# ByeongKyuPark/Depth-Aware-Shader-Effects-for-NeRF

Hardware: AMD Instinct MI355X
Metric: rays/sec at 800x800, 64 coarse + 128 fine samples (higher is better)
Workload: dtype fp32 (f16x3 split)

## Files before the change

### depth-aware-shader-effects-for-nerf_amd/csrc/mlp16s.hip

```cpp
#include <atomic>
#include "common.h"
#include "pe_sin.h"
#include "stream16.h"

namespace nerf {

#ifdef NERF_MLP16S_STAMPS
__device__ unsigned long long nerf16s_stamps[65536][16];
constexpr int kSStampFloats = kW16Waves * 32;
constexpr int kSStampIter = 8;
#define STAMP16S_ASM(i, insn)                                                               \
  do {                                                                                      \
    __builtin_amdgcn_sched_barrier(0);                                                      \
    unsigned long long t_;                                                                  \
    asm volatile(insn " %0\n\ts_waitcnt lgkmcnt(0)" : "=s"(t_)::"memory");                 \
    __builtin_amdgcn_sched_barrier(0);                                                      \
    if (lane == 0 && stamp_on) reinterpret_cast<unsigned long long*>(lds + kSLdsFloats)[wave * 16 + (i)] = t_; \
  } while (0)
#define STAMP16S(i) STAMP16S_ASM(i, "s_memtime")
#define STAMP16S_REAL(i) STAMP16S_ASM(i, "s_memrealtime")
#else
constexpr int kSStampFloats = 0;
#define STAMP16S(i) do {} while (0)
#define STAMP16S_REAL(i) do {} while (0)
#endif

__device__ __forceinline__ f32x4 mfma16s(h16x8 a, h16x8 b, f32x4 c) {
  return __builtin_amdgcn_mfma_f32_16x16x32_f16(a, b, c, 0, 0, 0);
}

constexpr int kSLdsPe = 4 * kChunkFloats;
constexpr int kSLdsBias = kSLdsPe + kW16Waves * kPeSteps * 64;
constexpr int kSLdsSigmaW = kSLdsBias + 8 * kHidden;
constexpr int kSLdsVecFloats = 8 * kHidden + kHidden + 4;
constexpr int kSLdsConsts = kSLdsBias + kSLdsVecFloats;
constexpr int kSLdsRgb = kSLdsConsts + kS16Consts;
constexpr int kSLdsRgbFloats = 3 * kDirHidden + 4;
constexpr int kSLdsFeat = kSLdsRgb + kSLdsRgbFloats;
constexpr int kSLdsFloats = kSLdsFeat + kW16Waves * kRayFeat;
static_assert(kSLdsRgb % 4 == 0 && kSLdsFeat % 4 == 0, "LDS vector layout");
static_assert((kS16Chunks & (kS16Chunks - 1)) == 0 && kS16Chunks % 4 == 0, "the stream wraps onto the same ring slots");

typedef h16x8 STile[2][2];
typedef f32x4 SAcc[8][2][2];

template <int TI>
__device__ __forceinline__ void sread_tile(const float* slot, const uint32_t (&off)[2], STile& a) {
#pragma unroll
  for (int r = 0; r < 2; ++r)
#pragma unroll
    for (int part = 0; part < 2; ++part)
      a[r][part] = __builtin_bit_cast(h16x8, *reinterpret_cast<const f32x4*>(slot + off[r] + TI * 512 + part * 256));
}

template <int G, int TI, bool FIRST, typename Hook>
__device__ __forceinline__ void smfma_tile(const STile& a, const Operand& b0, const Operand& b1, SAcc& acc,
                                           Hook&& hook) {
  static_for<4>([&](auto jc) __attribute__((always_inline)) {
    constexpr int j = decltype(jc)::value, r = j >> 1, st = j & 1;
    const Operand& b = st ? b1 : b0;
    f32x4 c;
    if constexpr (FIRST) c = mfma16s(a[r][1], b.hi, f32x4{});
    else c = mfma16s(a[r][1], b.hi, acc[4 * G + TI][r][st]);
    c = mfma16s(a[r][0], b.lo, c);
    acc[4 * G + TI][r][st] = mfma16s(a[r][0], b.hi, c);
    hook(jc);
  });
}

constexpr int kSValuGap0 = 5;
template <int G, int TI, bool FIRST, int NRD, int VPG, typename Reads, typename Side, typename Hook>
__device__ __forceinline__ void ssegment(const STile& a, const Operand& b0, const Operand& b1, SAcc& acc, Reads&& reads,
                                         Side&& side, Hook&& hook) {
  side(std::integral_constant<int, 0>{});
  __builtin_amdgcn_sched_barrier(0);
  reads();
  smfma_tile<G, TI, FIRST>(a, b0, b1, acc, hook);
  side(std::integral_constant<int, 1>{});
#pragma unroll
  for (int i = 0; i < 12; ++i) {
    __builtin_amdgcn_sched_group_barrier(0x008, 1, 0);
    if (i >= 1 && i <= 4 * NRD) __builtin_amdgcn_sched_group_barrier(0x100, 1, 0);
    if (VPG > 0 && i >= kSValuGap0) __builtin_amdgcn_sched_group_barrier(0x002, VPG, 0);
  }
  __builtin_amdgcn_sched_barrier(0);
}

enum SSide { kSNone, kSPrev, kSCur, kSL0, kSSkipPrev, kSSkipCur, kSPrevPe, kSCurPe };
__device__ __forceinline__ constexpr int spe_at(int i, int seg) {
  return (i == 7 || i == 8) && (seg == 0 || seg == 2) ? 2 * (i - 7) + seg / 2 : -1;
}
__device__ __forceinline__ constexpr int sq_prev(int i, int seg) {
  constexpr int base[7] = {0, 3, 6, 8, 10, 12, 14};
  if (i >= 7) return -1;
  const int n = i < 2 ? 3 : 2;
  if (n == 3) return seg >= 1 ? base[i] + seg - 1 : -1;
  return seg == 1 ? base[i] : (seg == 3 ? base[i] + 1 : -1);
}
__device__ __forceinline__ constexpr int sq_cur(int i, int seg) {
  constexpr int base[8] = {0, 0, 2, 4, 6, 8, 11, 14};
  constexpr int cnt[8] = {0, 2, 2, 2, 2, 3, 3, 2};
  if (i >= 8 || cnt[i] == 0) return -1;
  if (cnt[i] == 3) return seg >= 1 ? base[i] + seg - 1 : -1;
  return seg == 1 ? base[i] : (seg == 3 ? base[i] + 1 : -1);
}
template <bool CUR>
__device__ __forceinline__ constexpr int spe_next(int i, int seg) {
  if (i >= 8 || (CUR ? sq_cur(i, seg) : sq_prev(i, seg)) >= 0) return -1;
  int n = 0;
  for (int k = 0; k < 4 * i + seg; ++k) n += (CUR ? sq_cur(k / 4, k % 4) : sq_prev(k / 4, k % 4)) < 0;
  return n + (CUR ? 0 : 16);
}
static_assert(spe_next<true>(7, 2) == 15 && spe_next<false>(7, 3) == 31, "32 free segments");
template <int KIND>
__device__ __forceinline__ constexpr int side_count(int i, int seg) {
  if constexpr (KIND == kSPrevPe || KIND == kSCurPe) return 1;
  if constexpr (KIND == kSPrev) return sq_prev(i, seg) >= 0;
  if constexpr (KIND == kSSkipPrev) return (sq_prev(i, seg) >= 0) + (spe_at(i, seg) >= 0);
  if constexpr (KIND == kSCur) return sq_cur(i, seg) >= 0;
  if constexpr (KIND == kSSkipCur) return (sq_cur(i, seg) >= 0) + (spe_at(i, seg) >= 0);
  if constexpr (KIND == kSL0) return 2;
  return 0;
}
template <int KIND>
__device__ __forceinline__ constexpr int svpg(int i, int seg) {
  const int n = side_count<KIND>(i, seg);
  return n == 0 ? 0 : (n * 40 + 11 - kSValuGap0) / (12 - kSValuGap0);
}

struct SNoPub {
  template <typename I>
  __device__ __forceinline__ void operator()(I) const {}
};
template <int G, int SLOT, bool FIRST, int TAIL, int KIND, int I, bool WRAP, typename Side, typename Pub>
__device__ __forceinline__ void schunk(const float* __restrict__ stream, int c, float* lds, uint32_t lds_dma,
                                       uint32_t voff, const uint32_t (&off)[2], STile (&a)[4], const Operand& b0,
                                       const Operand& b1, SAcc& acc, Side&& side, Pub&& pub) {
  const float* cur = lds + SLOT * kChunkFloats;
  const float* nxt = lds + ((SLOT + 1) & 3) * kChunkFloats;
  auto none = [](auto) {};
  auto sd = [&side](auto seg_c) __attribute__((always_inline)) {
    return [&side, seg_c](auto ph) __attribute__((always_inline)) { side(std::integral_constant<int, I>{}, seg_c, ph); };
  };
  using S0 = std::integral_constant<int, 0>;
  using S1 = std::integral_constant<int, 1>;
  using S2 = std::integral_constant<int, 2>;
  using S3 = std::integral_constant<int, 3>;
  ssegment<G, 0, FIRST, 1, svpg<KIND>(I, 0)>(a[0], b0, b1, acc, [&]() __attribute__((always_inline)) {
    sread_tile<3>(cur, off, a[3]);
  }, sd(S0{}), none);
  if constexpr (TAIL >= 1) {
    wait_vmcnt<TAIL >= 2 ? 4 : 0>();
    __builtin_amdgcn_s_barrier();
  }
  pub(std::integral_constant<int, I>{});
  auto dma = [&](auto pc) __attribute__((always_inline)) {
    if constexpr (TAIL >= 3)
      chunk_dma_piece<(SLOT + 3) & 3, decltype(pc)::value>(stream, WRAP ? (c + 3) & (kS16Chunks - 1) : c + 3, lds_dma,
                                                           voff);
  };
  ssegment<G, 1, FIRST, (TAIL >= 1), svpg<KIND>(I, 1)>(a[1], b0, b1, acc, [&]() __attribute__((always_inline)) {
    if constexpr (TAIL >= 1) sread_tile<0>(nxt, off, a[0]);
  }, sd(S1{}), [&](auto jc) __attribute__((always_inline)) {
    if constexpr (decltype(jc)::value == 0) dma(S0{});
    if constexpr (decltype(jc)::value == 2) dma(S1{});
  });
  ssegment<G, 2, FIRST, (TAIL >= 1), svpg<KIND>(I, 2)>(a[2], b0, b1, acc, [&]() __attribute__((always_inline)) {
    if constexpr (TAIL >= 1) sread_tile<1>(nxt, off, a[1]);
  }, sd(S2{}), [&](auto jc) __attribute__((always_inline)) {
    if constexpr (decltype(jc)::value == 0) dma(S2{});
  });
  ssegment<G, 3, FIRST, (TAIL >= 1), svpg<KIND>(I, 3)>(a[3], b0, b1, acc, [&]() __attribute__((always_inline)) {
    if constexpr (TAIL >= 1) sread_tile<2>(nxt, off, a[2]);
  }, sd(S3{}), [&](auto jc) __attribute__((always_inline)) {
    if constexpr (decltype(jc)::value == 0) dma(S3{});
  });
}

template <int G, int NSTEP, int SLOT0, int TAIL_END, int KIND, bool WRAP = false, typename Opnd, typename Side,
          typename Pub = SNoPub>
__device__ __forceinline__ void sgroup(const float* __restrict__ stream, int c0, float* lds, uint32_t lds_dma,
                                       uint32_t voff, const uint32_t (&off)[2], STile (&a)[4], SAcc& acc,
                                       Opnd&& operand, Side&& side, Pub&& pub = Pub{}) {
  static_for<NSTEP>([&](auto ic) __attribute__((always_inline)) {
    constexpr int i = decltype(ic)::value;
    constexpr int left = NSTEP - 1 - i + TAIL_END;
    schunk<G, (SLOT0 + i) & 3, i == 0, (left < 3 ? left : 3), KIND, i, WRAP>(
        stream, c0 + i, lds, lds_dma, voff, off, a, operand(ic, std::integral_constant<int, 0>{}),
        operand(ic, std::integral_constant<int, 1>{}), acc, side, pub);
  });
}

__device__ __forceinline__ float smax4(float m) {
  m = fmaxf(m, __shfl_xor(m, 16));
  return fmaxf(m, __shfl_xor(m, 32));
}
__device__ __forceinline__ float ssum4(float v) {
  v = v + __shfl_xor(v, 16);
  return v + __shfl_xor(v, 32);
}

struct SQuarter {
  f32x4 b, w;
};

template <int PH, int T0, int QG, bool SIGMA>
__device__ __forceinline__ void squarter(const SAcc& acc, const float (&inv)[2], const float* bias, const float* ws,
                                         int nlane, const float (&sc)[2], Operand (&in)[16], float (&m)[2],
                                         float (&part)[2], SQuarter& qv) {
  constexpr int T = T0 + QG / 4, r = (QG % 4) >> 1, st = QG & 1;
  const int n0 = 32 * T + 8 * r + nlane;
  if constexpr (PH == 0) {
    qv.b = *reinterpret_cast<const f32x4*>(bias + n0);
    if constexpr (SIGMA) qv.w = *reinterpret_cast<const f32x4*>(ws + n0);
  } else {
    float xs[4];
#pragma unroll
    for (int e = 0; e < 4; ++e) {
      const float y = fmaxf(fmaf(acc[T][r][st][e], inv[st], qv.b[e]), 0.0f);
      m[st] = fmaxf(m[st], y);
      if constexpr (SIGMA) part[st] = fmaf(qv.w[e], y, part[st]);
      xs[e] = y * sc[st];
    }
    Operand& op = in[2 * T + st];
    typedef _Float16 h16x2 __attribute__((ext_vector_type(2)));
#pragma unroll
    for (int p = 0; p < 2; ++p) {
      const h16x2 hi2 = {(_Float16)xs[2 * p], (_Float16)xs[2 * p + 1]};
      const h16x2 lo2 = __builtin_bit_cast(h16x2, split_lo_pair(__builtin_bit_cast(uint32_t, hi2), xs[2 * p], xs[2 * p + 1]));
      const int j = 4 * r + 2 * p;
      op.hi[j] = hi2[0];
      op.hi[j + 1] = hi2[1];
      op.lo[j] = lo2[0];
      op.lo[j + 1] = lo2[1];
    }
  }
}

template <int PH, int t, int st>
__device__ __forceinline__ void spe_operand(const float* pe_mine, const float (&sc)[2], Operand& op, float (&v)[8],
                                            int lane) {
  if constexpr (PH == 0) {
#pragma unroll
    for (int j = 0; j < 8; ++j) v[j] = pe_mine[((st * 2 + t) * 8 + j) * 64 + lane];
  } else {
#pragma unroll
    for (int j = 0; j < 8; ++j) split_into(v[j] * sc[st], op, j);
  }
}

#define MLP16S_GATHER 0
#include "mlp16s_body.h"
#undef MLP16S_GATHER
#define MLP16S_GATHER 1
#include "mlp16s_body.h"
#undef MLP16S_GATHER

static int device_cus() {
  static std::atomic<int> cached[64];
  int dev = 0;
  if (hipGetDevice(&dev) != hipSuccess || dev < 0 || dev >= 64) return 0;
  int n = cached[dev].load(std::memory_order_relaxed);
  if (n == 0) {
    if (hipDeviceGetAttribute(&n, hipDeviceAttributeMultiprocessorCount, dev) != hipSuccess || n <= 0) return 0;
    cached[dev].store(n, std::memory_order_relaxed);
  }
  return n;
}

int launch_mlp16s(const float* packed, const float* o, const float* d, const float* z, int64_t R, int N,
                  const float* feat, float* rgb, float* sigma, const int* out_slot, int out_T, hipStream_t s) {
  const int64_t M = R * (int64_t)N;
  if (M == 0) return NERF_OK;
  constexpr int per_block = 32 * kW16Waves;
  const int64_t blocks = (M + per_block - 1) / per_block;
  const int cus = device_cus();
  if (cus <= 0) return set_error(NERF_ERR_HIP, "mlp16s_kernel: cannot read the device's CU count");
  hipLaunchKernelGGL(mlp16s_kernel, dim3((unsigned)(blocks < cus ? blocks : cus)), dim3(64 * kW16Waves), 0, s, packed, o, d, z, M, N, feat,
                     rgb, sigma, out_slot, out_T);
  return check_launch("mlp16s_kernel");
}

int launch_mlp16s_live(const float* packed, const float* o, const float* d, const float* z, int64_t R, int N,
                       const float* feat, float* rgb, float* sigma, const int* live, const int* live_count,
                       hipStream_t s) {
  const int64_t M = R * (int64_t)N;
  if (M == 0) return NERF_OK;
  constexpr int per_block = 32 * kW16Waves;
  const int64_t blocks = (M + per_block - 1) / per_block;
  const int cus = device_cus();
  if (cus <= 0) return set_error(NERF_ERR_HIP, "mlp16s_live_kernel: cannot read the device's CU count");
  hipLaunchKernelGGL(mlp16s_live_kernel, dim3((unsigned)(blocks < cus ? blocks : cus)), dim3(64 * kW16Waves), 0, s,
                     packed, o, d, z, N, feat, rgb, sigma, live, live_count);
  return check_launch("mlp16s_live_kernel");
}

}
```

### depth-aware-shader-effects-for-nerf_amd/csrc/mlp16s_body.h

```cpp
__global__ void __launch_bounds__(64 * kW16Waves, 1)
#if MLP16S_GATHER
mlp16s_live_kernel(const float* __restrict__ packed, const float* __restrict__ orig, const float* __restrict__ dirs,
                   const float* __restrict__ zv, int N, const float* __restrict__ feat, float* __restrict__ rgb,
                   float* __restrict__ sigma, const int* __restrict__ live, const int* __restrict__ live_count) {
#else
mlp16s_kernel(const float* __restrict__ packed, const float* __restrict__ orig, const float* __restrict__ dirs,
              const float* __restrict__ zv, int64_t M, int N, const float* __restrict__ feat,
              float* __restrict__ rgb, float* __restrict__ sigma, const int* __restrict__ out_slot, int out_T) {
#endif
  __shared__ __attribute__((aligned(16))) float lds[kSLdsFloats + kSStampFloats];
  const int wave = __builtin_amdgcn_readfirstlane(threadIdx.x >> 6), lane0 = threadIdx.x & 63;
#if MLP16S_GATHER
  const int64_t M = *live_count;
  if ((int64_t)blockIdx.x * (32 * kW16Waves) >= M) return;
  const int* const out_slot = nullptr;
  constexpr int out_T = 0;
#endif
  const int mlast = (int)(M - 1);
  const int nblk = (int)((M + 32 * kW16Waves - 1) / (32 * kW16Waves));
  int blk = blockIdx.x;
  auto sample_of = [&](int b, int st) {
    return imin64(((int64_t)b * kW16Waves + wave) * 32 + 16 * st + (lane0 & 15), (int64_t)mlast);
  };
  float in_z[2], in_o[2][3], in_d[2][3];
#if MLP16S_GATHER
  int sm_cur[2], sm_n[2];
  auto load_live = [&](int b, int (&sm)[2]) __attribute__((always_inline)) {
#pragma unroll
    for (int st = 0; st < 2; ++st) sm[st] = live[sample_of(b, st)];
  };
  auto load_inputs = [&](const int (&sml)[2]) __attribute__((always_inline)) {
#pragma unroll
    for (int st = 0; st < 2; ++st) {
      const int sm = sml[st];
#else
  auto load_inputs = [&](int b) __attribute__((always_inline)) {
#pragma unroll
    for (int st = 0; st < 2; ++st) {
      const int sm = (int)sample_of(b, st);
#endif
      const int64_t row = zv ? sm / N : sm;
#pragma unroll
      for (int c = 0; c < 3; ++c) in_o[st][c] = orig[3 * row + c];
      in_z[st] = 0.0f;
#pragma unroll
      for (int c = 0; c < 3; ++c) in_d[st][c] = 0.0f;
      if (zv) {
        in_z[st] = zv[sm];
#pragma unroll
        for (int c = 0; c < 3; ++c) in_d[st][c] = dirs[3 * row + c];
      }
    }
  };
  float x[2][3];
  auto positions = [&](float (&x)[2][3]) __attribute__((always_inline)) {
#pragma unroll
    for (int st = 0; st < 2; ++st)
#pragma unroll
      for (int c = 0; c < 3; ++c) {
        const float p = in_o[st][c] + in_d[st][c] * in_z[st];
        x[st][c] = zv ? p : in_o[st][c];
      }
  };
#if MLP16S_GATHER
  load_live(blk, sm_cur);
  load_inputs(sm_cur);
#else
  load_inputs(blk);
#endif
  positions(x);
  for (int i = threadIdx.x; i < kSLdsVecFloats / 4; i += 64 * kW16Waves)
    reinterpret_cast<f32x4*>(lds + kSLdsBias)[i] = reinterpret_cast<const f32x4*>(packed + kOffBias)[i];
  if (threadIdx.x < kS16Consts) lds[kSLdsConsts + threadIdx.x] = packed[kOffScale16 + threadIdx.x];
  if (threadIdx.x < kSLdsRgbFloats / 4)
    reinterpret_cast<f32x4*>(lds + kSLdsRgb)[threadIdx.x] = reinterpret_cast<const f32x4*>(packed + kOffRgbW)[threadIdx.x];
  __builtin_amdgcn_s_waitcnt(0);
  __builtin_amdgcn_sched_barrier(0);
  const float* stream = packed + kOff16;
  uint32_t lds_dma = (uint32_t)(uintptr_t)(lptr_t)lds + 1024u * wave;
  auto fragment_offsets = [](int l, uint32_t (&off)[2]) __attribute__((always_inline)) {
    const int li = l & 15, hh = (l >> 4) & 1, ss = l >> 5;
#pragma unroll
    for (int r = 0; r < 2; ++r) off[r] = (uint32_t)(ss * 2048 + 4 * ((li & 7) + 8 * r + 16 * (li >> 3) + 32 * hh));
  };
  float* pe_mine = lds + kSLdsPe + wave * kPeSteps * 64;
  const float* bias = lds + kSLdsBias;
  const float* ws = lds + kSLdsSigmaW;
  const float* cst = lds + kSLdsConsts;
#if MLP16S_GATHER
  constexpr bool one_ray = false;
#else
  const bool one_ray = (N & 31) == 0;
#endif
  float* feat_mine = lds + kSLdsFeat + wave * kRayFeat;
  STile a[4];
  {
    const uint32_t voff = 16u * lane0 + 1024u * wave;
    chunk_dma<0>(stream, 0, lds_dma, voff);
    chunk_dma<1>(stream, 1, lds_dma, voff);
    chunk_dma<2>(stream, 2, lds_dma, voff);
    uint32_t off[2];
    fragment_offsets(lane0, off);
    wait_vmcnt<8>();
    __builtin_amdgcn_s_barrier();
    sread_tile<0>(lds, off, a[0]);
    sread_tile<1>(lds, off, a[1]);
    sread_tile<2>(lds, off, a[2]);
  }

  Operand pe_op[4];
  bool full = true;
#ifdef NERF_MLP16S_STAMPS
  int it = 0;
#endif
#pragma unroll 1
  for (;;) {
  asm volatile("" : "+s"(stream));
  asm volatile("" : "+s"(lds_dma));
  int lane = lane0;
  asm volatile("" : "+v"(lane));
  const int g = lane >> 4, li = lane & 15, hh = g & 1, ss = g >> 1;
  const uint32_t voff = 16u * lane + 1024u * wave;
  uint32_t off[2];
  fragment_offsets(lane, off);
  const int nlane = 4 * hh + 16 * ss;
#ifdef NERF_MLP16S_STAMPS
  const bool stamp_on = it == kSStampIter || (it < kSStampIter && blk + (int)gridDim.x >= nblk);
  ++it;
#endif
  STAMP16S(0);
  STAMP16S_REAL(12);
  const int64_t s0 = ((int64_t)blk * kW16Waves + wave) * 32;

  auto pe_arg = [&](const float (&xa)[2][3], int st, int p) __attribute__((always_inline)) {
    const int fi = p / 3, fc = p - 3 * fi;
    const float xc = fc == 0 ? xa[st][0] : (fc == 1 ? xa[st][1] : xa[st][2]);
    return xc * __int_as_float((127 + (fi < kPosLevels ? fi : 0)) << 23);
  };
  auto pe_tail = [&](const float (&xa)[2][3], int st, int p, float v) __attribute__((always_inline)) {
    return p < 3 * kPosLevels ? v : (p == 30 ? (hh ? xa[st][1] : xa[st][0]) : (hh ? 0.0f : xa[st][2]));
  };
  auto pe_beyond = [&](const float (&xa)[2][3]) __attribute__((always_inline)) {
    float ax = 0.0f;
#pragma unroll
    for (int st = 0; st < 2; ++st)
      ax = fmaxf(ax, fmaxf(fabsf(xa[st][0]), fmaxf(fabsf(xa[st][1]), fabsf(xa[st][2]))));
    return __any(ax * (float)(1 << (kPosLevels - 1)) > kPeSinMax) != 0;
  };
  auto pe_bound = [&](const float (&xa)[2][3], int st) __attribute__((always_inline)) {
    return fmaxf(1.0f, fmaxf(fabsf(xa[st][0]), fmaxf(fabsf(xa[st][1]), fabsf(xa[st][2]))));
  };
  float m_pe[2];
  float s_cur[2], inv_cur[2], s_nxt[2], inv_prev[2], m[2] = {0.0f, 0.0f}, part[2] = {0.0f, 0.0f};
#pragma unroll
  for (int st = 0; st < 2; ++st) {
    m_pe[st] = pe_bound(x, st);
    s_cur[st] = pow2_scale(m_pe[st]);
  }
  if (full) {
    float pe[2][2][8];
    if (pe_beyond(x)) {
#pragma unroll
      for (int st = 0; st < 2; ++st)
#pragma unroll
        for (int t = 0; t < 2; ++t)
#pragma unroll
          for (int j = 0; j < 8; ++j) {
            const int p = 8 * (2 * t + ss) + j;
            float sn, cs;
            sincosf(pe_arg(x, st, p), &sn, &cs);
            pe[st][t][j] = pe_tail(x, st, p, hh ? cs : sn);
          }
    } else {
#pragma unroll
      for (int st = 0; st < 2; ++st)
#pragma unroll
        for (int t = 0; t < 2; ++t)
#pragma unroll
          for (int j = 0; j < 8; ++j) {
            const int p = 8 * (2 * t + ss) + j;
            pe[st][t][j] = pe_tail(x, st, p, pe_sin_reduced(pe_arg(x, st, p), hh));
          }
    }
#pragma unroll
    for (int st = 0; st < 2; ++st)
#pragma unroll
      for (int t = 0; t < 2; ++t)
#pragma unroll
        for (int j = 0; j < 8; ++j) {
          pe_mine[((st * 2 + t) * 8 + j) * 64 + lane] = pe[st][t][j];
          split_into(pe[st][t][j] * s_cur[st], pe_op[2 * t + st], j);
        }
  }
  const int nxt_blk = blk + (int)gridDim.x;
  float xn[2][3], s_n[2];
  bool beyond_n = false;
  Operand pe_nx[4];
  int lane_n = lane;
  auto pub_next = [&](auto ic) __attribute__((always_inline)) {
#if MLP16S_GATHER
    if constexpr (decltype(ic)::value == 0) load_live(nxt_blk, sm_n);
    if constexpr (decltype(ic)::value == 1) load_inputs(sm_n);
    if constexpr (decltype(ic)::value == 3) {
#else
    if constexpr (decltype(ic)::value == 0) load_inputs(nxt_blk);
    if constexpr (decltype(ic)::value == 2) {
#endif
      asm volatile("" : "+v"(lane_n));
      positions(xn);
#pragma unroll
      for (int st = 0; st < 2; ++st) s_n[st] = pow2_scale(pe_bound(xn, st));
      beyond_n = pe_beyond(xn);
    }
  };
  auto side_pe_next = [&](auto nc, auto ph) __attribute__((always_inline)) {
    constexpr int n = decltype(nc)::value;
    if constexpr (n >= 0 && decltype(ph)::value == 1) {
      constexpr int st = n >> 4, t = (n >> 3) & 1, j = n & 7;
      constexpr int p0 = 16 * t + j, p1 = p0 + 8;
      constexpr int f0 = p0 / 3, c0 = p0 % 3, f1 = p1 / 3 < kPosLevels ? p1 / 3 : 0, c1 = p1 % 3;
      const bool upper = lane_n >= 32;
      const int hn = (lane_n >> 4) & 1;
      const float a0 = xn[st][c0] * (float)(1 << f0), a1 = xn[st][c1] * (float)(1 << f1);
      const float r = pe_sin_reduced(upper ? a1 : a0, hn);
      float v = r;
      if constexpr (p1 == 30) v = upper ? (hn ? xn[st][1] : xn[st][0]) : r;
      if constexpr (p1 == 31) v = upper ? (hn ? 0.0f : xn[st][2]) : r;
      pe_mine[((st * 2 + t) * 8 + j) * 64 + lane_n] = v;
      split_into(v * s_n[st], pe_nx[2 * t + st], j);
      asm volatile("" : "+v"(pe_nx[2 * t + st].hi), "+v"(pe_nx[2 * t + st].lo));
    }
  };
  SAcc acc;
  Operand in[16];
#pragma unroll
  for (int st = 0; st < 2; ++st) {
    inv_cur[st] = cst[kS16InvW + 0] / s_cur[st];
    s_nxt[st] = pow2_scale(cst[kS16R + 0] * m_pe[st] + cst[kS16B + 0]);
  }
  SQuarter qv[2];
  float pe_v[8];
  auto pe_operand_of = [&](auto i, auto st) -> const Operand& {
    return pe_op[2 * decltype(i)::value + decltype(st)::value];
  };

  STAMP16S(1);
  sgroup<0, 2, 0, 3, kSNone>(stream, 0, lds, lds_dma, voff, off, a, acc, pe_operand_of,
                             [](auto, auto, auto) {});
  sgroup<1, 2, 2, 3, kSL0>(stream, 2, lds, lds_dma, voff, off, a, acc, pe_operand_of,
                           [&](auto i, auto seg, auto ph) __attribute__((always_inline)) {
                             constexpr int q0 = 8 * decltype(i)::value + 2 * decltype(seg)::value;
                             squarter<decltype(ph)::value, 0, q0, false>(acc, inv_cur, bias, ws, nlane, s_nxt, in, m,
                                                                         part, qv[0]);
                             squarter<decltype(ph)::value, 0, q0 + 1, false>(acc, inv_cur, bias, ws, nlane, s_nxt, in,
                                                                             m, part, qv[1]);
                           });

  STAMP16S(2);
#pragma unroll
  for (int st = 0; st < 2; ++st) {
    inv_prev[st] = inv_cur[st];
    s_cur[st] = s_nxt[st];
  }
  const float* bias_prev = bias;
  auto act_operand = [&](auto i, auto st) -> const Operand& { return in[2 * decltype(i)::value + decltype(st)::value]; };
  auto op4 = [&](auto i, auto st) -> const Operand& {
    constexpr int k = decltype(i)::value, t = decltype(st)::value;
    if constexpr (k < 8) return in[2 * k + t];
    else return pe_op[2 * (k - 8) + t];
  };
  auto side_prev = [&](auto i, auto seg, auto ph, auto sigma_tag) __attribute__((always_inline)) {
    constexpr int q = sq_prev(decltype(i)::value, decltype(seg)::value);
    if constexpr (q >= 0)
      squarter<decltype(ph)::value, 4, q, decltype(sigma_tag)::value>(acc, inv_prev, bias_prev, ws, nlane, s_cur, in, m,
                                                                       part, qv[0]);
  };
  auto side_cur = [&](auto i, auto seg, auto ph, const float* bias_l, auto sigma_tag) __attribute__((always_inline)) {
    constexpr int q = sq_cur(decltype(i)::value, decltype(seg)::value);
    if constexpr (q >= 0)
      squarter<decltype(ph)::value, 0, q, decltype(sigma_tag)::value>(acc, inv_cur, bias_l, ws, nlane, s_nxt, in, m,
                                                                      part, qv[1]);
  };
  float s_pe[2] = {0.0f, 0.0f};
  auto side_pe = [&](auto i, auto seg, auto ph) __attribute__((always_inline)) {
    constexpr int k = spe_at(decltype(i)::value, decltype(seg)::value);
    if constexpr (k >= 0) spe_operand<decltype(ph)::value, k / 2, k % 2>(pe_mine, s_pe, pe_op[k], pe_v, lane);
  };
  using NoSigma = std::false_type;
  using Sigma = std::true_type;
  auto layer = [&](int L, auto skip_tag, auto sg_tag, auto&& pub_a) __attribute__((always_inline)) {
    constexpr bool SKIP = decltype(skip_tag)::value;
    constexpr bool SG = decltype(sg_tag)::value;
#pragma unroll
    for (int st = 0; st < 2; ++st) {
      inv_cur[st] = cst[kS16InvW + L] / s_cur[st];
      if constexpr (SKIP) s_pe[st] = s_cur[st];
    }
    const float* bias_l = bias + L * kHidden;
    const int c0 = s16_chunk0(1) + (L - 1) * 16 + (L > kSkipLayer ? 4 : 0);
    if constexpr (SKIP) {
      sgroup<0, 10, 0, 3, kSSkipPrev>(stream, c0, lds, lds_dma, voff, off, a, acc, op4,
                                      [&](auto i, auto seg, auto ph) __attribute__((always_inline)) {
                                        side_prev(i, seg, ph, NoSigma{});
                                        side_pe(i, seg, ph);
                                      });
    } else {
      sgroup<0, 8, 0, 3, kSPrev>(stream, c0, lds, lds_dma, voff, off, a, acc, act_operand,
                                 [&](auto i, auto seg, auto ph) __attribute__((always_inline)) {
                                   side_prev(i, seg, ph, NoSigma{});
                                 }, pub_a);
    }
#pragma unroll
    for (int st = 0; st < 2; ++st) {
      const float ms = smax4(m[st]);
      float bound = cst[kS16R + L] * (SKIP ? fmaxf(ms, m_pe[st]) : ms) + cst[kS16B + L];
      if (L + 1 == kSkipLayer) bound = fmaxf(bound, m_pe[st]);
      s_nxt[st] = pow2_scale(bound);
      m[st] = 0.0f;
    }
    if constexpr (SKIP) {
      sgroup<1, 10, 2, 3, kSSkipCur>(stream, c0 + 10, lds, lds_dma, voff, off, a, acc, op4,
                                     [&](auto i, auto seg, auto ph) __attribute__((always_inline)) {
                                       side_cur(i, seg, ph, bias_l, NoSigma{});
                                       side_pe(i, seg, ph);
                                     });
    } else {
      sgroup<1, 8, 0, 3, SG ? kSCurPe : kSCur>(
          stream, c0 + 8, lds, lds_dma, voff, off, a, acc, act_operand,
          [&](auto i, auto seg, auto ph) __attribute__((always_inline)) {
            side_cur(i, seg, ph, bias_l, sg_tag);
            if constexpr (SG)
              side_pe_next(std::integral_constant<int, spe_next<true>(decltype(i)::value, decltype(seg)::value)>{}, ph);
          });
    }
#pragma unroll
    for (int st = 0; st < 2; ++st) {
      inv_prev[st] = inv_cur[st];
      s_cur[st] = s_nxt[st];
    }
    bias_prev = bias_l;
    STAMP16S(2 + L);
  };
#pragma unroll 1
  for (int L = 1; L < kSkipLayer; ++L) layer(L, NoSigma{}, NoSigma{}, SNoPub{});
  layer(kSkipLayer, Sigma{}, NoSigma{}, SNoPub{});
#pragma unroll 1
  for (int L = kSkipLayer + 1; L < 7; ++L) layer(L, NoSigma{}, NoSigma{}, SNoPub{});
  layer(7, NoSigma{}, Sigma{}, pub_next);

  if (one_ray) {
    const char* src = reinterpret_cast<const char*>(feat + (imin64(s0, M - 1) / N) * kRayFeat);
    const uint32_t dst = (uint32_t)(uintptr_t)(lptr_t)feat_mine;
    uint32_t keep;
    asm volatile(
        "s_mov_b32 %0, m0\n\t"
        "s_mov_b32 m0, %3\n\t"
        "s_nop 0\n\t"
        "global_load_lds_dwordx4 %1, %2\n\t"
        "s_mov_b32 m0, %0"
        : "=&s"(keep)
        : "v"(16u * lane), "s"(src), "s"(dst)
        : "memory");
  }
#pragma unroll
  for (int st = 0; st < 2; ++st) inv_cur[st] = cst[kS16InvW + 8] / s_cur[st];
  sgroup<0, 8, 0, 3, kSPrevPe, true>(
      stream, s16_chunk0(8), lds, lds_dma, voff, off, a, acc, act_operand,
      [&](auto i, auto seg, auto ph) __attribute__((always_inline)) {
        side_prev(i, seg, ph, Sigma{});
        side_pe_next(std::integral_constant<int, spe_next<false>(decltype(i)::value, decltype(seg)::value)>{}, ph);
      });

  STAMP16S(10);
  float sig[2];
#pragma unroll
  for (int st = 0; st < 2; ++st) sig[st] = fmaxf(ssum4(part[st]) + ws[kHidden], 0.0f);
  const float* wr = lds + kSLdsRgb;
  float pr[2][3] = {{0.0f, 0.0f, 0.0f}, {0.0f, 0.0f, 0.0f}};
  auto colour_head = [&](const float* fr, int st) __attribute__((always_inline)) {
#pragma unroll
    for (int T = 0; T < 4; ++T)
#pragma unroll
      for (int r = 0; r < 2; ++r) {
        const int n0 = 32 * T + 8 * r + nlane;
        const f32x4 fd = *reinterpret_cast<const f32x4*>(fr + n0);
        const f32x4 ap = *reinterpret_cast<const f32x4*>(fr + kDirHidden + n0);
        f32x4 hd;
#pragma unroll
        for (int e = 0; e < 4; ++e) hd[e] = fmaxf(fmaf(acc[T][r][st][e], inv_cur[st], fd[e]), 0.0f) + ap[e];
#pragma unroll
        for (int c = 0; c < 3; ++c) {
          const f32x4 w = *reinterpret_cast<const f32x4*>(wr + c * kDirHidden + n0);
#pragma unroll
          for (int e = 0; e < 4; ++e) pr[st][c] = fmaf(w[e], hd[e], pr[st][c]);
        }
      }
  };
  if (one_ray) wait_vmcnt<8>();
  if (one_ray) {
    colour_head(feat_mine, 0);
    colour_head(feat_mine, 1);
  } else {
#if MLP16S_GATHER
    colour_head(feat + (int64_t)(sm_cur[0] / N) * kRayFeat, 0);
    colour_head(feat + (int64_t)(sm_cur[1] / N) * kRayFeat, 1);
#else
    colour_head(feat + (int64_t)((int)sample_of(blk, 0) / N) * kRayFeat, 0);
    colour_head(feat + (int64_t)((int)sample_of(blk, 1) / N) * kRayFeat, 1);
#endif
  }
  float out[3];
#pragma unroll
  for (int c = 0; c < 3; ++c) {
    const float v0 = ssum4(pr[0][c]) + wr[3 * kDirHidden + c], v1 = ssum4(pr[1][c]) + wr[3 * kDirHidden + c];
    const float v = (g & 1) ? v1 : v0;
    out[c] = 1.0f / (1.0f + expf_rn(-v));
  }
  if (g < 2) {
    const int st = g;
    if (s0 + 16 * st + li < M) {
#if MLP16S_GATHER
      const int sm = st ? sm_cur[1] : sm_cur[0];
#else
      const int sm = (int)(s0 + 16 * st + li);
#endif
      const int64_t o_s = out_slot ? (int64_t)(sm / N) * out_T + out_slot[sm] : (int64_t)sm;
      sigma[o_s] = st ? sig[1] : sig[0];
#pragma unroll
      for (int c = 0; c < 3; ++c) rgb[3 * o_s + c] = out[c];
    }
  }
  STAMP16S(11);
  STAMP16S_REAL(13);
  if (nxt_blk >= nblk) break;
  blk = nxt_blk;
  full = beyond_n;
#pragma unroll
  for (int k = 0; k < 4; ++k) pe_op[k] = pe_nx[k];
#pragma unroll
  for (int st = 0; st < 2; ++st)
#pragma unroll
    for (int c = 0; c < 3; ++c) x[st][c] = xn[st][c];
#if MLP16S_GATHER
  sm_cur[0] = sm_n[0];
  sm_cur[1] = sm_n[1];
#endif
  }
  wait_vmcnt<0>();
#ifdef NERF_MLP16S_STAMPS
  if (const int64_t w_ = (int64_t)blockIdx.x * kW16Waves + wave; w_ < 65536 && lane0 == 0)
    for (int i = 0; i < 16; ++i)
      nerf16s_stamps[w_][i] = reinterpret_cast<const unsigned long long*>(lds + kSLdsFloats)[wave * 16 + i];
#endif
}
```

Measured before the change: 2.267 million.

## Interleave half-quarter epilogue work and fragment reads between individual MFMAs

Adds a finer-grained segment scheduler that splits each layer's activation epilogue (bias, ReLU, scale, fp16 split) into six-step half-quarter units. These units are placed between individual MFMA instructions using per-instruction sched barriers, and tile reads are split into per-fragment LDS loads. By default it also replaces the four piece DMA per chunk with wave-wide global_load_lds_dwordx4 issued per wave at a larger stride. The aim is to hide VALU and LDS latency under matrix work and cut DMA issue overhead, at the cost of a more rigid schedule and different LDS staging per wave.

```diff
diff --git a/depth-aware-shader-effects-for-nerf_amd/csrc/mlp16s.hip b/depth-aware-shader-effects-for-nerf_amd/csrc/mlp16s.hip
--- a/depth-aware-shader-effects-for-nerf_amd/csrc/mlp16s.hip
+++ b/depth-aware-shader-effects-for-nerf_amd/csrc/mlp16s.hip
@@ -53,6 +53,43 @@
       a[r][part] = __builtin_bit_cast(h16x8, *reinterpret_cast<const f32x4*>(slot + off[r] + TI * 512 + part * 256));
 }
 
+template <int TI, int K>
+__device__ __forceinline__ void sread_frag(const float* slot, const uint32_t (&off)[2], STile& a) {
+  constexpr int r = K >> 1, part = K & 1;
+  a[r][part] = __builtin_bit_cast(h16x8, *reinterpret_cast<const f32x4*>(slot + off[r] + TI * 512 + part * 256));
+}
+
+#ifdef NERF16S_PIECE_DMA
+constexpr uint32_t kSDmaWave = 1024;
+template <int SLOT, int I>
+__device__ __forceinline__ void sdma_piece(const float* __restrict__ stream, int c, uint32_t lds_base, uint32_t voff) {
+  chunk_dma_piece<SLOT, I>(stream, c, lds_base, voff);
+}
+#else
+constexpr uint32_t kSDmaWave = 4096;
+template <int SLOT, int I>
+__device__ __forceinline__ void sdma_piece(const float* __restrict__ stream, int c, uint32_t lds_base, uint32_t voff) {
+  const char* src = reinterpret_cast<const char*>(stream) + (size_t)c * (kChunkFloats * 4);
+  if constexpr (I == 0)
+    asm volatile(
+        "s_mov_b32 m0, %2\n\t"
+        "s_nop 0\n\t"
+        "global_load_lds_dwordx4 %0, %1"
+        :
+        : "v"(voff), "s"(src), "s"(lds_base + SLOT * (kChunkFloats * 4))
+        : "memory", "m0");
+  else
+    asm volatile("global_load_lds_dwordx4 %0, %1 offset:%2" : : "v"(voff), "s"(src), "n"(I * 1024) : "memory");
+}
+#endif
+template <int SLOT>
+__device__ __forceinline__ void sdma_chunk(const float* __restrict__ stream, int c, uint32_t lds_base, uint32_t voff) {
+  sdma_piece<SLOT, 0>(stream, c, lds_base, voff);
+  sdma_piece<SLOT, 1>(stream, c, lds_base, voff);
+  sdma_piece<SLOT, 2>(stream, c, lds_base, voff);
+  sdma_piece<SLOT, 3>(stream, c, lds_base, voff);
+}
+
 template <int G, int TI, bool FIRST, typename Hook>
 __device__ __forceinline__ void smfma_tile(const STile& a, const Operand& b0, const Operand& b1, SAcc& acc,
                                            Hook&& hook) {
@@ -86,7 +123,36 @@
   __builtin_amdgcn_sched_barrier(0);
 }
 
-enum SSide { kSNone, kSPrev, kSCur, kSL0, kSSkipPrev, kSSkipCur, kSPrevPe, kSCurPe };
+__device__ __forceinline__ constexpr int shalf_unit_at(int gap, int slot, bool two) {
+  if (two) return gap >= 5 + slot && gap <= 10 + slot ? gap - 5 - slot : -2;
+  return slot ? -2 : (gap >= 5 && gap <= 7 ? gap - 5 : (gap >= 9 && gap <= 11 ? gap - 6 : -2));
+}
+template <int G, int TI, bool FIRST, int NRD, bool TWO, typename Frag, typename Side, typename Hook>
+__device__ __forceinline__ void ssegment_h(const STile& a, const Operand& b0, const Operand& b1, SAcc& acc, Frag&& frag,
+                                           Side&& side, Hook&& hook) {
+  using Slot0 = std::integral_constant<int, 0>;
+  using Slot1 = std::integral_constant<int, 1>;
+  side(Slot0{}, std::integral_constant<int, -1>{});
+  side(Slot1{}, std::integral_constant<int, -1>{});
+  __builtin_amdgcn_sched_barrier(0);
+  static_for<12>([&](auto ic) __attribute__((always_inline)) {
+    constexpr int i = decltype(ic)::value, j = i / 3, k = i % 3, r = j >> 1, st = j & 1;
+    const Operand& b = st ? b1 : b0;
+    f32x4& c = acc[4 * G + TI][r][st];
+    if constexpr (k == 0) c = FIRST ? mfma16s(a[r][1], b.hi, f32x4{}) : mfma16s(a[r][1], b.hi, c);
+    if constexpr (k == 1) c = mfma16s(a[r][0], b.lo, c);
+    if constexpr (k == 2) {
+      c = mfma16s(a[r][0], b.hi, c);
+      hook(std::integral_constant<int, j>{});
+    }
+    if constexpr (i >= 1 && i <= 4 * NRD) frag(std::integral_constant<int, i - 1>{});
+    side(Slot0{}, std::integral_constant<int, shalf_unit_at(i, 0, TWO)>{});
+    side(Slot1{}, std::integral_constant<int, shalf_unit_at(i, 1, TWO)>{});
+    __builtin_amdgcn_sched_barrier(0);
+  });
+}
+
+enum SSide { kSNone, kSPrev, kSCur, kSL0, kSSkipPrev, kSSkipCur, kSPrevPe, kSCurPe, kSPrevH, kSCurH };
 __device__ __forceinline__ constexpr int spe_at(int i, int seg) {
   return (i == 7 || i == 8) && (seg == 0 || seg == 2) ? 2 * (i - 7) + seg / 2 : -1;
 }
@@ -104,6 +170,26 @@
   if (cnt[i] == 3) return seg >= 1 ? base[i] + seg - 1 : -1;
   return seg == 1 ? base[i] : (seg == 3 ? base[i] + 1 : -1);
 }
+__device__ __forceinline__ constexpr int sh_prev(int i, int seg, int slot) {
+  if (i == 0) return 2 * seg + slot;
+  return i >= 7 || slot ? -1 : 8 + 4 * (i - 1) + seg;
+}
+__device__ __forceinline__ constexpr int sh_cur(int i, int seg, int slot) {
+  if (i == 7) return 24 + 2 * seg + slot;
+  return i == 0 || i >= 8 || slot ? -1 : 4 * (i - 1) + seg;
+}
+__device__ __forceinline__ constexpr bool sh_schedules_hold() {
+  int np = 0, nc = 0;
+  for (int i = 0; i < 8; ++i)
+    for (int seg = 0; seg < 4; ++seg)
+      for (int slot = 0; slot < 2; ++slot) {
+        const int hp = sh_prev(i, seg, slot), hc = sh_cur(i, seg, slot);
+        if (hp >= 0 && (hp != np++ || i >= 4 + hp / 8)) return false;
+        if (hc >= 0 && (hc != nc++ || i <= hc / 8)) return false;
+      }
+  return np == 32 && nc == 32;
+}
+static_assert(sh_schedules_hold(), "half-quarter schedules: each half once, in order, inside its window");
 template <bool CUR>
 __device__ __forceinline__ constexpr int spe_next(int i, int seg) {
   if (i >= 8 || (CUR ? sq_cur(i, seg) : sq_prev(i, seg)) >= 0) return -1;
@@ -126,6 +212,23 @@
 __device__ __forceinline__ constexpr int svpg(int i, int seg) {
   const int n = side_count<KIND>(i, seg);
   return n == 0 ? 0 : (n * 40 + 11 - kSValuGap0) / (12 - kSValuGap0);
+}
+
+template <int G, int TI, bool FIRST, int NRD, int KIND, int I, typename Frag, typename Side, typename Hook>
+__device__ __forceinline__ void sseg(const STile& a, const Operand& b0, const Operand& b1, SAcc& acc, Frag&& frag,
+                                     Side&& side, Hook&& hook) {
+  using IC = std::integral_constant<int, I>;
+  using SC = std::integral_constant<int, TI>;
+  if constexpr (KIND == kSPrevH || KIND == kSCurH) {
+    constexpr bool two = (KIND == kSPrevH ? sh_prev(I, TI, 1) : sh_cur(I, TI, 1)) >= 0;
+    ssegment_h<G, TI, FIRST, NRD, two>(a, b0, b1, acc, frag, [&](auto slot, auto unit) __attribute__((always_inline)) {
+      side(IC{}, SC{}, slot, unit);
+    }, hook);
+  } else {
+    ssegment<G, TI, FIRST, NRD, svpg<KIND>(I, TI)>(a, b0, b1, acc, [&]() __attribute__((always_inline)) {
+      static_for<4>(frag);
+    }, [&](auto ph) __attribute__((always_inline)) { side(IC{}, SC{}, ph); }, hook);
+  }
 }
 
 struct SNoPub {
@@ -139,16 +242,13 @@
   const float* cur = lds + SLOT * kChunkFloats;
   const float* nxt = lds + ((SLOT + 1) & 3) * kChunkFloats;
   auto none = [](auto) {};
-  auto sd = [&side](auto seg_c) __attribute__((always_inline)) {
-    return [&side, seg_c](auto ph) __attribute__((always_inline)) { side(std::integral_constant<int, I>{}, seg_c, ph); };
-  };
   using S0 = std::integral_constant<int, 0>;
   using S1 = std::integral_constant<int, 1>;
   using S2 = std::integral_constant<int, 2>;
   using S3 = std::integral_constant<int, 3>;
-  ssegment<G, 0, FIRST, 1, svpg<KIND>(I, 0)>(a[0], b0, b1, acc, [&]() __attribute__((always_inline)) {
-    sread_tile<3>(cur, off, a[3]);
-  }, sd(S0{}), none);
+  sseg<G, 0, FIRST, 1, KIND, I>(a[0], b0, b1, acc, [&](auto kc) __attribute__((always_inline)) {
+    sread_frag<3, decltype(kc)::value>(cur, off, a[3]);
+  }, side, none);
   if constexpr (TAIL >= 1) {
     wait_vmcnt<TAIL >= 2 ? 4 : 0>();
     __builtin_amdgcn_s_barrier();
@@ -156,23 +256,22 @@
   pub(std::integral_constant<int, I>{});
   auto dma = [&](auto pc) __attribute__((always_inline)) {
     if constexpr (TAIL >= 3)
-      chunk_dma_piece<(SLOT + 3) & 3, decltype(pc)::value>(stream, WRAP ? (c + 3) & (kS16Chunks - 1) : c + 3, lds_dma,
-                                                           voff);
+      sdma_piece<(SLOT + 3) & 3, decltype(pc)::value>(stream, WRAP ? (c + 3) & (kS16Chunks - 1) : c + 3, lds_dma, voff);
   };
-  ssegment<G, 1, FIRST, (TAIL >= 1), svpg<KIND>(I, 1)>(a[1], b0, b1, acc, [&]() __attribute__((always_inline)) {
-    if constexpr (TAIL >= 1) sread_tile<0>(nxt, off, a[0]);
-  }, sd(S1{}), [&](auto jc) __attribute__((always_inline)) {
+  sseg<G, 1, FIRST, (TAIL >= 1), KIND, I>(a[1], b0, b1, acc, [&](auto kc) __attribute__((always_inline)) {
+    if constexpr (TAIL >= 1) sread_frag<0, decltype(kc)::value>(nxt, off, a[0]);
+  }, side, [&](auto jc) __attribute__((always_inline)) {
     if constexpr (decltype(jc)::value == 0) dma(S0{});
     if constexpr (decltype(jc)::value == 2) dma(S1{});
   });
-  ssegment<G, 2, FIRST, (TAIL >= 1), svpg<KIND>(I, 2)>(a[2], b0, b1, acc, [&]() __attribute__((always_inline)) {
-    if constexpr (TAIL >= 1) sread_tile<1>(nxt, off, a[1]);
-  }, sd(S2{}), [&](auto jc) __attribute__((always_inline)) {
+  sseg<G, 2, FIRST, (TAIL >= 1), KIND, I>(a[2], b0, b1, acc, [&](auto kc) __attribute__((always_inline)) {
+    if constexpr (TAIL >= 1) sread_frag<1, decltype(kc)::value>(nxt, off, a[1]);
+  }, side, [&](auto jc) __attribute__((always_inline)) {
     if constexpr (decltype(jc)::value == 0) dma(S2{});
   });
-  ssegment<G, 3, FIRST, (TAIL >= 1), svpg<KIND>(I, 3)>(a[3], b0, b1, acc, [&]() __attribute__((always_inline)) {
-    if constexpr (TAIL >= 1) sread_tile<2>(nxt, off, a[2]);
-  }, sd(S3{}), [&](auto jc) __attribute__((always_inline)) {
+  sseg<G, 3, FIRST, (TAIL >= 1), KIND, I>(a[3], b0, b1, acc, [&](auto kc) __attribute__((always_inline)) {
+    if constexpr (TAIL >= 1) sread_frag<2, decltype(kc)::value>(nxt, off, a[2]);
+  }, side, [&](auto jc) __attribute__((always_inline)) {
     if constexpr (decltype(jc)::value == 0) dma(S3{});
   });
 }
@@ -235,6 +334,63 @@
       op.lo[j + 1] = lo2[1];
     }
   }
+}
+
+__device__ __forceinline__ void sunpaired(float& v, float after) {
+#ifndef NERF16S_PACKED_SIDE
+  asm("" : "+v"(v) : "v"(after));
+#endif
+}
+
+typedef float f32x2s __attribute__((ext_vector_type(2)));
+struct SHalf {
+  f32x2s b;
+  float y[2], xs[2];
+};
+
+template <int U, int T0, int H>
+__device__ __forceinline__ void shalf(const SAcc& acc, const float (&inv)[2], const float* bias, int nlane,
+                                      const float (&sc)[2], Operand (&in)[16], float (&m)[2], SHalf& hv) {
+  constexpr int QG = H >> 1, p = H & 1, T = T0 + QG / 4, r = (QG % 4) >> 1, st = QG & 1, j = 4 * r + 2 * p;
+  typedef _Float16 h16x2 __attribute__((ext_vector_type(2)));
+  Operand& op = in[2 * T + st];
+  if constexpr (U == -1) hv.b = *reinterpret_cast<const f32x2s*>(bias + 32 * T + 8 * r + nlane + 2 * p);
+  if constexpr (U == 0) {
+    hv.y[0] = fmaf(acc[T][r][st][2 * p], inv[st], hv.b[0]);
+    float b1 = hv.b[1];
+    sunpaired(b1, hv.y[0]);
+    hv.b[1] = b1;
+  }
+  if constexpr (U == 1) {
+    hv.y[1] = fmaf(acc[T][r][st][2 * p + 1], inv[st], hv.b[1]);
+    hv.y[0] = fmaxf(hv.y[0], 0.0f);
+  }
+  if constexpr (U == 2) {
+    hv.y[1] = fmaxf(hv.y[1], 0.0f);
+    hv.xs[0] = hv.y[0] * sc[st];
+    sunpaired(hv.y[1], hv.xs[0]);
+  }
+  if constexpr (U == 3) {
+    hv.xs[1] = hv.y[1] * sc[st];
+    m[st] = fmaxf(fmaxf(m[st], hv.y[0]), hv.y[1]);
+  }
+  if constexpr (U == 4) {
+    const h16x2 hi2 = {(_Float16)hv.xs[0], (_Float16)hv.xs[1]};
+    op.hi[j] = hi2[0];
+    op.hi[j + 1] = hi2[1];
+  }
+  if constexpr (U == 5) {
+    const h16x2 hi2 = {op.hi[j], op.hi[j + 1]};
+    const h16x2 lo2 = __builtin_bit_cast(h16x2, split_lo_pair(__builtin_bit_cast(uint32_t, hi2), hv.xs[0], hv.xs[1]));
+    op.lo[j] = lo2[0];
+    op.lo[j + 1] = lo2[1];
+  }
+}
+
+template <int U>
+__device__ __forceinline__ void shalf_follow(const SHalf& first, SHalf& second) {
+  if constexpr (U == 1) sunpaired(second.y[0], first.xs[0]);
+  if constexpr (U == 2) sunpaired(second.y[1], first.xs[1]);
 }
 
 template <int PH, int t, int st>
diff --git a/depth-aware-shader-effects-for-nerf_amd/csrc/mlp16s_body.h b/depth-aware-shader-effects-for-nerf_amd/csrc/mlp16s_body.h
--- a/depth-aware-shader-effects-for-nerf_amd/csrc/mlp16s_body.h
+++ b/depth-aware-shader-effects-for-nerf_amd/csrc/mlp16s_body.h
@@ -77,7 +77,7 @@
   __builtin_amdgcn_s_waitcnt(0);
   __builtin_amdgcn_sched_barrier(0);
   const float* stream = packed + kOff16;
-  uint32_t lds_dma = (uint32_t)(uintptr_t)(lptr_t)lds + 1024u * wave;
+  uint32_t lds_dma = (uint32_t)(uintptr_t)(lptr_t)lds + kSDmaWave * wave;
   auto fragment_offsets = [](int l, uint32_t (&off)[2]) __attribute__((always_inline)) {
     const int li = l & 15, hh = (l >> 4) & 1, ss = l >> 5;
 #pragma unroll
@@ -95,10 +95,10 @@
   float* feat_mine = lds + kSLdsFeat + wave * kRayFeat;
   STile a[4];
   {
-    const uint32_t voff = 16u * lane0 + 1024u * wave;
-    chunk_dma<0>(stream, 0, lds_dma, voff);
-    chunk_dma<1>(stream, 1, lds_dma, voff);
-    chunk_dma<2>(stream, 2, lds_dma, voff);
+    const uint32_t voff = 16u * lane0 + kSDmaWave * wave;
+    sdma_chunk<0>(stream, 0, lds_dma, voff);
+    sdma_chunk<1>(stream, 1, lds_dma, voff);
+    sdma_chunk<2>(stream, 2, lds_dma, voff);
     uint32_t off[2];
     fragment_offsets(lane0, off);
     wait_vmcnt<8>();
@@ -120,7 +120,7 @@
   int lane = lane0;
   asm volatile("" : "+v"(lane));
   const int g = lane >> 4, li = lane & 15, hh = g & 1, ss = g >> 1;
-  const uint32_t voff = 16u * lane + 1024u * wave;
+  const uint32_t voff = 16u * lane + kSDmaWave * wave;
   uint32_t off[2];
   fragment_offsets(lane, off);
   const int nlane = 4 * hh + 16 * ss;
@@ -239,6 +239,7 @@
     s_nxt[st] = pow2_scale(cst[kS16R + 0] * m_pe[st] + cst[kS16B + 0]);
   }
   SQuarter qv[2];
+  SHalf hv[2];
   float pe_v[8];
   auto pe_operand_of = [&](auto i, auto st) -> const Operand& {
     return pe_op[2 * decltype(i)::value + decltype(st)::value];
@@ -281,6 +282,25 @@
       squarter<decltype(ph)::value, 0, q, decltype(sigma_tag)::value>(acc, inv_cur, bias_l, ws, nlane, s_nxt, in, m,
                                                                       part, qv[1]);
   };
+  auto side_prev_h = [&](auto i, auto seg, auto slot, auto unit) __attribute__((always_inline)) {
+    constexpr int h = sh_prev(decltype(i)::value, decltype(seg)::value, decltype(slot)::value);
+    if constexpr (h >= 0 && decltype(unit)::value >= -1)
+      shalf<decltype(unit)::value, 4, h>(acc, inv_prev, bias_prev, nlane, s_cur, in, m, hv[decltype(slot)::value]);
+    if constexpr (decltype(slot)::value == 1 && h >= 0)
+      shalf_follow<decltype(unit)::value>(hv[0], hv[1]);
+  };
+  auto side_cur_h = [&](auto i, auto seg, auto slot, auto unit, const float* bias_l) __attribute__((always_inline)) {
+    constexpr int h = sh_cur(decltype(i)::value, decltype(seg)::value, decltype(slot)::value);
+    if constexpr (h >= 0 && decltype(unit)::value >= -1)
+      shalf<decltype(unit)::value, 0, h>(acc, inv_cur, bias_l, nlane, s_nxt, in, m, hv[decltype(slot)::value]);
+    if constexpr (decltype(slot)::value == 1 && h >= 0)
+      shalf_follow<decltype(unit)::value>(hv[0], hv[1]);
+  };
+#ifdef NERF16S_QUARTER_SIDE
+  constexpr int kKindPrev = kSPrev, kKindCur = kSCur;
+#else
+  constexpr int kKindPrev = kSPrevH, kKindCur = kSCurH;
+#endif
   float s_pe[2] = {0.0f, 0.0f};
   auto side_pe = [&](auto i, auto seg, auto ph) __attribute__((always_inline)) {
     constexpr int k = spe_at(decltype(i)::value, decltype(seg)::value);
@@ -305,10 +325,11 @@
                                         side_pe(i, seg, ph);
                                       });
     } else {
-      sgroup<0, 8, 0, 3, kSPrev>(stream, c0, lds, lds_dma, voff, off, a, acc, act_operand,
-                                 [&](auto i, auto seg, auto ph) __attribute__((always_inline)) {
-                                   side_prev(i, seg, ph, NoSigma{});
-                                 }, pub_a);
+      sgroup<0, 8, 0, 3, kKindPrev>(stream, c0, lds, lds_dma, voff, off, a, acc, act_operand,
+                                    [&](auto i, auto seg, auto... at) __attribute__((always_inline)) {
+                                      if constexpr (sizeof...(at) == 2) side_prev_h(i, seg, at...);
+                                      else side_prev(i, seg, at..., NoSigma{});
+                                    }, pub_a);
     }
 #pragma unroll
     for (int st = 0; st < 2; ++st) {
@@ -325,12 +346,17 @@
                                        side_pe(i, seg, ph);
                                      });
     } else {
-      sgroup<1, 8, 0, 3, SG ? kSCurPe : kSCur>(
+      sgroup<1, 8, 0, 3, SG ? kSCurPe : kKindCur>(
           stream, c0 + 8, lds, lds_dma, voff, off, a, acc, act_operand,
-          [&](auto i, auto seg, auto ph) __attribute__((always_inline)) {
-            side_cur(i, seg, ph, bias_l, sg_tag);
-            if constexpr (SG)
-              side_pe_next(std::integral_constant<int, spe_next<true>(decltype(i)::value, decltype(seg)::value)>{}, ph);
+          [&](auto i, auto seg, auto... at) __attribute__((always_inline)) {
+            if constexpr (sizeof...(at) == 2) {
+              side_cur_h(i, seg, at..., bias_l);
+            } else {
+              side_cur(i, seg, at..., bias_l, sg_tag);
+              if constexpr (SG)
+                side_pe_next(std::integral_constant<int, spe_next<true>(decltype(i)::value, decltype(seg)::value)>{},
+                             at...);
+            }
           });
     }
 #pragma unroll
```

Result: faster. 2.316 million (median of 6 runs) (+2.2%).
